# kensung-lab/hypo

Measured on AMD Instinct MI355X. Metric: polished windows/sec (whole node), higher is better.
Workload: dtype int16

## Files before the change

hypo_amd/csrc/poa_core.hpp:

```cpp
#pragma once
#include <math.h>
#include <type_traits>
#include "grp.hpp"
#include "../../include/hypo_gpu.h"

namespace hypo {
#ifdef HYPO_EMU_DBG
static unsigned long g_dbg_reason[16];
static unsigned long g_dbg_hist[64];
#define DBGH(d) do { if (g.lane == 0) g_dbg_hist[(d) < 63 ? (d) : 63]++; } while (0)
#else
#define DBGH(d) do { } while (0)
#endif

enum { MODE_NW = 1, MODE_LOV = 3, MODE_ROV = 4 };
enum { C_A = 0, C_C = 1, C_G = 2, C_T = 3, C_N = 4, C_J = 5, C_O = 6, C_NONE = 7 };
enum { PH_LOAD = 0, PH_DP = 1, PH_TRACE = 2, PH_ADD = 3, PH_TOPO = 4, PH_CONS = 5, PH_OUT = 6, PH_META = 7, PH_EXACT = 8, PH_N = 9 };
#if defined(HYPO_PHASE_TIMERS) && !defined(HYPO_EMU)
#define HYPO_TICK(k) do { const uint64_t t1_ = (uint64_t)clock64(); tphase[k] += t1_ - tlast; tlast = t1_; } while (0)
#define HYPO_TICK_RESET() do { tlast = (uint64_t)clock64(); } while (0)
#else
#define HYPO_TICK(k) do { } while (0)
#define HYPO_TICK_RESET() do { } while (0)
#endif

enum { RES_OK = 0, RES_OVERFLOW = 1, RES_UNDEFINED = 2, RES_CONS_OVERFLOW = 3, RES_UNSUPPORTED = 4, RES_INVALID = 5 };

struct PoaParams {
    const HypoWindow* windows;
    const uint8_t* draft4;
    const uint64_t* arm_off;
    const uint32_t* arm_len;
    const uint8_t* arms2;
    char* out_bases;
    const uint64_t* out_off;
    uint32_t* out_len;
    uint8_t* out_status;
    int sr_m, sr_n, sr_g, lr_m, lr_n, lr_g;
    uint64_t n_arms, draft4_bytes, arms2_bytes;
    int flags;
};
enum { POA_NATIVE_KLOV = 1, POA_MIN_CLASS_SHIFT = 8 };

#ifdef HYPO_EMU
struct PoaParamRef {
    const PoaParams* p;
    HD const PoaParams* operator->() const { return p; }
};
#else
struct PoaParamRef {
    typedef const PoaParams __attribute__((address_space(4)))* cptr;
    cptr p;
    HD cptr operator->() const { cptr q = p; asm volatile("" : "+s"(q)); return q; }
};
#endif

#ifndef HYPO_EXACT
#define HYPO_EXACT 1
#endif
#define HYPO_EXACT_WIDE 1
#ifndef HYPO_ONE_SUB
#define HYPO_ONE_SUB 1
#endif
#ifndef HYPO_ONE_SUB_ROV
#define HYPO_ONE_SUB_ROV 1
#endif
#ifndef HYPO_TOPO_INSERT
#define HYPO_TOPO_INSERT 1
#endif
#ifndef HYPO_DEFER_META
#define HYPO_DEFER_META 1
#endif
#define HYPO_PACKED 1
template <int GW_, int CPL_, int LCAP_, int NMAX_, int KIN_, int DIRCELLS_, int RINGCELLS_, int ARMBYTES_,
// ... 107 lines not shown
    static constexpr bool NIB = Cfg::NIB;
    static constexpr int NEG = -(1 << 29);
    static constexpr bool PK = Cfg::PACKED;
    static_assert(!PK || Cfg::NIB, "packed rows store nibble codes");
    static_assert(!PK || (int)sizeof(score_t) * Cfg::RINGCELLS >= Cfg::STK * (int)sizeof(id_t), "packed classes: the DFS stack fits the score ring");
    static constexpr int DIR_FAST = NIB ? 15 : 0xFF;
    static constexpr int DIR_HORIZ = NIB ? 14 : 0xFE;
    HD static int dir_diag(int p) { return NIB ? p : (p << 1); }
    HD static int dir_vert(int p) { return NIB ? 7 + p : ((p << 1) | 1); }
    HD static bool is_vert(int d) { return NIB ? d >= 7 : (d & 1); }
    HD static int dir_pred(int d) { return NIB ? (d >= 7 ? d - 7 : d) : (d >> 1); }

    static constexpr int pow2_of(int x) { return x & -x; }
    struct alignas(pow2_of((int)sizeof(score_t) * CPL)) Pack { score_t v[CPL]; };
    struct alignas(pow2_of(NIB ? CPL / 2 : CPL)) DPack { uint8_t v[NIB ? CPL / 2 : CPL]; };
    HD static uint32_t seq_ent(uint32_t src, uint32_t len, bool head, bool tail, int mode, bool , int where) {
        const uint32_t mc = mode == MODE_NW ? 0u : (mode == MODE_LOV ? 1u : 2u);
        return (src & 0x3fffu) | (len << 16) | ((head ? 1u : 0u) << 26) | ((tail ? 1u : 0u) << 27) | (mc << 28) |
               ((uint32_t)where << 30);
    }

    const Grp<GW>& g;
    const PoaParamRef P;
    score_t* ring; uint8_t* dir; uint32_t* rowmeta; uint32_t* seqtab; wt_t* inw; int16_t* posnode;
    id_t *inp, *al, *r2n, *n2r, *stack;
    uint8_t *code, *nin, *nout, *nal, *mark, *seq, *armbuf;
    uint8_t* sidx;
    id_t* pathnodes; uint32_t* pathoff; uint16_t *pathlen, *pathmult, *msa; uint32_t* dstcnt; uint8_t* consbuf; id_t* predrows; score_t* ring1;
    id_t *r2n_alt, *n2r_alt, *newid; int16_t* newslot;
    bool lazy_on; int n_new;
    int n_paths, path_used, head_first;
    int n_nodes; int L; bool topo_dirty; bool meta_dirty;
    int tb_steps; int tb_fv;
    bool last_changed;
    bool weights_done;
    bool threaded;
    enum { ST_CELLS = 0, ST_ALIGNS, ST_REUSED, ST_XHITS, ST_CSCORED, ST_CEXACT, ST_XT, ST_XH, ST_NEED, ST_CKIND, ST_CS, ST_CCHAIN0, ST_CPASS, ST_ARMB, ST_OLEN, ST_N,
           ST_LASTX = ST_CPASS,
           ST_MAXD = ST_N, ST_NSORT,
           ACC_CELLS, ACC_ALIGNS, ACC_ABYTES, ACC_REUSED, ACC_THR, ACC_CSCORED, ACC_CTHR, ACC_NOK, ACC_NESC, ACC_NFAIL, ACC_NCARRIED, ACC_END,
           NX_W0 = ACC_END, NX_OFF = NX_W0 + 10, NX_WIDX = NX_OFF + 4, NX_CARRY, CUR_STATIC, CUR_OFF, NX_END = CUR_OFF + 4 };
    static constexpr uint32_t NX_NONE = 0xffffffffu;
    static_assert(sizeof(HypoWindow) == 40, "the prefetch moves the descriptor as ten words");
    static_assert(NX_END <= Lay::STAT_BYTES / 4 && ST_N <= GW && GW >= 16, "stat block");
    enum { CARRY_NONE = 0, CARRY_BEFORE = 1, CARRY_UNSORTED = 2 };
    static constexpr int RES_OVERFLOW_CLEAN = 64;
    uint32_t* stat;
    HD void stat_add(int k, uint32_t v) const { if (g.lane == 0) stat[k] += v; }
    HD void stat_set(int k, uint32_t v) const { if (g.lane == 0) stat[k] = v; }
    HD uint32_t stat_get(int k) const { return stat[k]; }
#if defined(HYPO_PHASE_TIMERS) || defined(HYPO_EMU)
#define HYPO_DIAG(x) do { x; } while (0)
    uint32_t rows_done, topo_runs, cons_serial, rows_slow, exact_tries, guided_hits, rows_scored_n, topo_dfs, topo_fast;
    uint32_t one_sub_hits, cols_hits, topo_inserts, lazy_updates, tie_sorts;
#else
#define HYPO_DIAG(x) do { } while (0)
#endif
    uint64_t tphase[PH_N]; uint64_t tlast;

    HD Poa(const Grp<GW>& g_, const PoaParamRef& P_, char* mem, char* fast = nullptr, char* dirg = nullptr) : g(g_), P(P_) {
        ring = (score_t*)(mem + Lay::oRing); dir = Cfg::DIRG ? (uint8_t*)dirg : (uint8_t*)(mem + Lay::oDir);
        rowmeta = (uint32_t*)(mem + Lay::oRowmeta); seqtab = (uint32_t*)(mem + Lay::oSeqtab);
        inw = (wt_t*)(mem + Lay::oInw);
        constexpr bool HYB = Cfg::HYBRID;
        posnode = (int16_t*)(HYB ? fast + Lay::fPosnode : mem + Lay::oPosnode);
        inp = (id_t*)(mem + Lay::oInp); al = (id_t*)(mem + Lay::oAl);
        r2n = (id_t*)(mem + Lay::oR2n); n2r = (id_t*)(mem + Lay::oN2r);
        stack = (id_t*)(HYB ? fast + Lay::fPosnode : (PK ? mem + Lay::oRing : mem + Lay::oPosnode)); code = (uint8_t*)(mem + Lay::oCode);
        nin = (uint8_t*)(HYB ? fast + Lay::fNin : mem + Lay::oNin); nout = (uint8_t*)(mem + Lay::oNout);
        nal = (uint8_t*)(HYB ? fast + Lay::fNal : mem + Lay::oNal); mark = (uint8_t*)(HYB ? fast + Lay::fMark : mem + Lay::oMark);
        seq = (uint8_t*)(HYB ? fast + Lay::fSeq : mem + Lay::oSeq); armbuf = (uint8_t*)(mem + Lay::oArms);
        sidx = mark;
        pathnodes = (id_t*)(mem + Lay::oPathNodes); pathoff = (uint32_t*)(mem + Lay::oPathOff);
        pathlen = (uint16_t*)(mem + Lay::oPathLen); pathmult = (uint16_t*)(mem + Lay::oPathMult);
        msa = (uint16_t*)(mem + Lay::oMsa); dstcnt = (uint32_t*)(mem + Lay::oDst); consbuf = (uint8_t*)(mem + Lay::oCons);
        predrows = (id_t*)(mem + Lay::oPredRows);
        r2n_alt = (id_t*)(mem + Lay::oR2nAlt); n2r_alt = (id_t*)(mem + Lay::oN2rAlt); newid = (id_t*)(mem + Lay::oNewId); newslot = (int16_t*)(mem + Lay::oNewSlot);
        if constexpr (Cfg::LAZY_RING) {
            constexpr int oA = align_up<2>((NMAX + 1) * 2 > Cfg::STK * (int)sizeof(id_t) ? (NMAX + 1) * 2 : Cfg::STK * (int)sizeof(id_t));
            constexpr int oB = oA + NMAX * (int)sizeof(id_t), oC = oB + NMAX * (int)sizeof(id_t), oD = align_up<2>(oC + (Cfg::LMAX + 1) * (int)sizeof(id_t));
            static_assert(oD + (Cfg::LMAX + 1) * 2 <= (int)sizeof(score_t) * Cfg::RINGCELLS, "the lazy order's scratch fits the score ring");
            r2n_alt = (id_t*)(mem + Lay::oRing + oA); n2r_alt = (id_t*)(mem + Lay::oRing + oB); newid = (id_t*)(mem + Lay::oRing + oC); newslot = (int16_t*)(mem + Lay::oRing + oD);
        }
        lazy_on = false; n_new = 0; guide_len = -1; guide_mode = 0;
        stat = (uint32_t*)(HYB ? fast + Lay::fStat : mem + Lay::oStat);
        for (int t = g.lane; t < Lay::STAT_BYTES / 4; t += GW) stat[t] = 0;
        ring1 = (score_t*)(HYB ? fast + Lay::fRing1 : mem + Lay::oRing);
        n_paths = 0; path_used = 0; head_first = 0;
        n_nodes = 0; L = 0; topo_dirty = false; meta_dirty = true; tb_steps = 0; tb_fv = 0;
        last_changed = true; threaded = false;
        HYPO_DIAG(rows_done = 0; topo_runs = 0; cons_serial = 0; rows_slow = 0; exact_tries = 0; guided_hits = 0; rows_scored_n = 0; topo_dfs = 0; topo_fast = 0; one_sub_hits = 0; cols_hits = 0; topo_inserts = 0; lazy_updates = 0; tie_sorts = 0);
        for (int i = 0; i < PH_N; ++i) tphase[i] = 0;
        tlast = 0;
        HYPO_TICK_RESET();
    }

    Hook hk;
    HD void fetch_next() const {
        if constexpr (Hook::enabled) {
            g.sync();
            uint32_t a = 0;
            if (g.lane == 0) a = hk.claim();
            const uint32_t count = hk.count();
            const uint32_t idx = (uint32_t)g.shfl((int)a, 0);
            const uint32_t wn = idx < count ? hk.item(idx) : NX_NONE;
            a = wn;
            if (wn != NX_NONE) {
                if (g.lane < 10) a = ((const uint32_t*)(P->windows + wn))[g.lane];
                else if (g.lane < 14) a = ((const uint32_t*)(P->out_off + wn))[g.lane - 10];
                else if (g.lane == 15) a = idx >= hk.planned() ? hk.carry(wn) : 0u;
            }
            if (g.lane < 16) stat[NX_W0 + g.lane] = a;
            g.sync();
        }
    }
    HD void out_range(uint32_t w, uint64_t* o, uint64_t* cap) const {
        if constexpr (Hook::enabled) {
            const uint64_t o0 = (uint64_t)stat[CUR_OFF] | ((uint64_t)stat[CUR_OFF + 1] << 32), o1 = (uint64_t)stat[CUR_OFF + 2] | ((uint64_t)stat[CUR_OFF + 3] << 32);
            *o = o0; *cap = o1 - o0;
        } else { *o = P->out_off[w]; *cap = P->out_off[w + 1] - *o; }
    }

    HD int build_seqtab(const HypoWindow& W, bool is_long, int* n_seq_out, bool* added_out) {
        const uint32_t a0 = W.first_arm;
        const int ni = (int)W.n_internal, np = (int)W.n_prefix, ns = (int)W.n_suffix;
        const int narm = ni + np + ns;
        const int base = (ni == 0 || is_long) ? 1 : 0;
        if (narm + base > Cfg::SEQMAX) return RES_OVERFLOW;
        if ((int)W.draft_len + (is_long ? 0 : 2) > Cfg::LMAX && base) return RES_OVERFLOW;
        g.sync();
        if (base && g.lane == 0) seqtab[0] = seq_ent(0, W.draft_len, !is_long, !is_long, MODE_NW, true, 2);
        bool over = false, any_len = false, bad = false;
        uint32_t armb = 0;
        if constexpr (STAGE_FUSED) {
            if (!is_long) return build_seqtab_fused(W, base, narm, n_seq_out, added_out);
        }
        for (int t = g.lane; t < narm; t += GW) {
            int a, mode; bool head, tail;
            if (is_long) { a = t; mode = MODE_NW; head = false; tail = false; }
            else if (t < ni) { a = t; mode = MODE_NW; head = true; tail = true; }
            else if (t < ni + np) { a = ni + (np - 1 - (t - ni)); mode = MODE_LOV; head = true; tail = false; }
            else { a = t; mode = MODE_ROV; head = false; tail = true; }
            const uint32_t len = P->arm_len[a0 + a];
            { const uint64_t ao = P->arm_off[a0 + a], ab = P->arms2_bytes; if (ao > ab || ((uint64_t)len + 3) / 4 > ab - ao) { bad = true; continue; } }
// ... 2415 lines not shown
                int c = 0;
                for (int q = 0; q < pl; ++q) {
                    const int v = pn[q];
                    const int mv = msa[v];
                    while (c < len && (int)msa[path[len - 1 - c]] < mv) ++c;
                    if (c >= len) break;
                    const int cn = path[len - 1 - c];
                    if ((int)msa[cn] == mv && code[v] == code[cn]) atomic_inc(&dstcnt[c], mult);
                }
            }
            g.sync();
            int o = 0;
            for (int base = 0; base < len; base += GW) {
                const int c = base + g.lane;
                const bool keep = c < len && counter_load(&dstcnt[c]) >= thr;
                const uint64_t kb = g.ballot(keep);
                const int cd = c < len ? (int)code[path[len - 1 - c]] : 0;
                g.sync();
                if (keep) consbuf[o + popc64(kb & ((1ull << g.lane) - 1ull))] = (uint8_t)cd;
                o += popc64(kb);
            }
            conslen = o;
            g.sync();
            HYPO_TICK(PH_CONS);
        }
        uint64_t oo, cap; out_range(w, &oo, &cap);
        if ((uint64_t)conslen > cap) { finish(w, HYPO_ST_CONS_OVERFLOW, (uint32_t)conslen); return RES_OK; }
        for (int t = g.lane; t < conslen; t += GW) P->out_bases[oo + t] = "ACGTNJO"[consbuf[t]];
        finish(w, HYPO_ST_OK, (uint32_t)conslen);
        return RES_OK;
    }

    HD void finish(uint32_t w, int status, uint32_t len) const {
        if (g.lane == 0) { P->out_len[w] = len; P->out_status[w] = (uint8_t)status; if constexpr (Hook::enabled) stat[ST_OLEN] = len; }
    }
    HD int emit_draft(uint32_t w, const uint8_t* d4, int dlen) const {
        uint64_t o, cap; out_range(w, &o, &cap);
        if ((uint64_t)dlen > cap) { finish(w, HYPO_ST_CONS_OVERFLOW, (uint32_t)dlen); return RES_OK; }
        for (int t = g.lane; t < dlen; t += GW) {
            int c = (d4[t >> 1] >> (4 - 4 * (t & 1))) & 15;
            P->out_bases[o + t] = "ACGTN"[c < 4 ? c : 4];
        }
        finish(w, HYPO_ST_OK, (uint32_t)dlen);
        return RES_OK;
    }

    HD int run_short(uint32_t w, const HypoWindow& W, const uint8_t* carry_in) {
        const int m = P->sr_m, n = P->sr_n, gp = P->sr_g;
        const uint8_t* d4 = P->draft4 + W.draft_off;
        n_nodes = 0; topo_dirty = false; meta_dirty = true;
        lazy_on = Cfg::LAZY && !Cfg::LAZY_RING && !(P->flags & POA_NATIVE_KLOV);
        stat_set(ST_NSORT, 0u);
        int n_seq = 0; bool added = false;
        int rc = build_seqtab(W, false, &n_seq, &added);
        if (rc != RES_OK) return rc;
        bool prev_aligned = false;
        int s = 0;
        int chain0_in = 0;
        if (carry_in) {
            if ((rc = restore(carry_in, &s, &chain0_in)) != RES_OK) return rc;
            if (s > n_seq) return RES_INVALID;
            if (topo_dirty) { if ((rc = toposort()) != RES_OK) return rc; HYPO_DIAG(topo_runs += 1); HYPO_TICK(PH_TOPO); }
            if constexpr (Cfg::LAZY_RING) { if (!(P->flags & POA_NATIVE_KLOV)) lazy_on = true; }
        }
        int chain0 = chain0_in;
        auto project = [&](int rc_) -> int {
            if (rc_ == RES_OVERFLOW && s > 0 && n_nodes > 0) {
                const int grown = n_nodes - chain0 > 0 ? n_nodes - chain0 : 0;
                if (g.lane == 0) {
                    stat[ST_NEED] = (uint32_t)(n_nodes + (int)(((int64_t)grown * (n_seq - s) + s - 1) / s) + 4);
                    const uint32_t kind = stat[ST_CKIND];
                    stat[ST_CS] = (uint32_t)(kind == CARRY_UNSORTED ? s : s - 1);
                    stat[ST_CCHAIN0] = (uint32_t)(chain0 ? chain0 : (kind == CARRY_UNSORTED ? n_nodes : 0));
                }
            } else stat_set(ST_CKIND, CARRY_NONE);
            g.sync();
            return rc_;
        };
        while (s < n_seq) {
            if (prev_aligned && !last_changed && tb_steps != 0 && tb_fv == 0) {
                int c = 0;
                while (s < n_seq && same_as_previous(s)) { ++c; ++s; }
                if (c) {
                    if (g.lane == 0) { stat[ST_CELLS] += (uint32_t)(c * (n_nodes + 1) * (L + 1)); stat[ST_ALIGNS] += c; stat[ST_REUSED] += c; }
                    if ((rc = readd_alignment(c)) != RES_OK) return project(rc);
                    HYPO_TICK(PH_ADD);
                    if (s >= n_seq) break;
                }
            }
            int mode;
            if ((rc = load_seq(W, s, &mode)) != RES_OK) return rc;
            ++s;
            if (L == 0) { prev_aligned = false; continue; }
            if ((rc = add_sequence_step(mode, m, n, gp)) != RES_OK) return project(rc);
            if (chain0 == 0) chain0 = n_nodes;
            prev_aligned = true;
        }
        if (!added) return emit_draft(w, d4, (int)W.draft_len);
        if constexpr (Cfg::LAZY) {
            if (lazy_on && n_nodes > 0) { if ((rc = toposort()) != RES_OK) return rc; meta_dirty = true; HYPO_TICK(PH_TOPO); }
            lazy_on = false;
        }
        int16_t* path;
        const int len = consensus(&path);
        HYPO_TICK(PH_CONS);
        if (len < 2) return RES_UNDEFINED;
        const int olen = len - 2;
        uint64_t o, cap; out_range(w, &o, &cap);
        if ((uint64_t)olen > cap) { finish(w, HYPO_ST_CONS_OVERFLOW, (uint32_t)olen); return RES_OK; }
        for (int t = g.lane; t < olen; t += GW) P->out_bases[o + t] = "ACGTNJO"[code[path[len - 2 - t]]];
        finish(w, HYPO_ST_OK, (uint32_t)olen);
        HYPO_TICK(PH_OUT);
        return RES_OK;
    }

    HD int run(uint32_t w, const uint8_t* carry_in = nullptr) {
        const HypoWindow W = P->windows[w];
        return run_window(w, W, carry_in);
    }
    HD int run_window(uint32_t w, const HypoWindow& W, const uint8_t* carry_in) {
        last_changed = true;
        g.sync();
        if (g.lane < ST_N) stat[g.lane] = 0;
        g.sync();
        HYPO_DIAG(rows_done = 0; topo_runs = 0; cons_serial = 0; rows_slow = 0; exact_tries = 0; guided_hits = 0; rows_scored_n = 0; topo_dfs = 0; topo_fast = 0; one_sub_hits = 0; cols_hits = 0; topo_inserts = 0; lazy_updates = 0; tie_sorts = 0);
        n_paths = 0; path_used = 0; head_first = 0; L = 0; tb_steps = 0; tb_fv = 0;
        lazy_on = false; n_new = 0; guide_len = -1;
        for (int i = 0; i < PH_N; ++i) tphase[i] = 0;
        HYPO_TICK_RESET();
        const uint32_t ne = W.n_internal + W.n_prefix + W.n_suffix;
        if ((uint64_t)W.n_internal + W.n_prefix + W.n_suffix > P->n_arms || (uint64_t)W.first_arm + ne > P->n_arms ||
            W.draft_off > P->draft4_bytes || ((uint64_t)W.draft_len + 1) / 2 > P->draft4_bytes - W.draft_off) return RES_INVALID;
        if constexpr (Hook::enabled) {
            if ((W.n_empty > ne || ne < 2) && g.lane == 0) {
                uint32_t a = 0;
                HYPO_NOUNROLL
                for (uint32_t t = 0; t < ne; ++t) a += (P->arm_len[W.first_arm + t] + 3) >> 2;
                stat[ST_ARMB] = a;
            }
        }
        if (W.n_empty > ne) { finish(w, HYPO_ST_OK, 0); return RES_OK; }
        if (ne < 2) return emit_draft(w, P->draft4 + W.draft_off, (int)W.draft_len);
        if (W.type != HYPO_WIN_SHORT) {
            if (Cfg::PATHCAP == 0) return RES_UNSUPPORTED;
            return run_long(w, W);
        }
        const int rc = run_short(w, W, carry_in);
        if (g.lane == 0) stat[ST_CPASS] = (rc == RES_OVERFLOW && carry_in && stat[ST_CKIND] == CARRY_NONE) ? 1u : 0u;
        g.sync();
        return rc;
    }
};

}
```

hypo_amd/csrc/poa_kernel.hip:

```cpp
#include <hip/hip_runtime.h>
#include <hip/hip_ext.h>
#include <atomic>
#include <stdio.h>
#include <stdlib.h>
#include "poa_classes.hpp"
#include "poa_kernel.hpp"
#include "poa_giant.hpp"
#include <cstring>

namespace hypo {

struct ClassLimits { int lmax, nmax, dircells, ringcells, seqmax, cpl; };

template <class Cfg> __host__ __device__ constexpr ClassLimits limits_of() {
    return ClassLimits{Cfg::LMAX, Cfg::NMAX, Cfg::DIRCELLS, Cfg::RINGCELLS, Cfg::SEQMAX, Cfg::CPL};
}

constexpr int PLAN_THREADS = 256;
constexpr int PLAN_STAGE = 4096;
constexpr int PLAN_AHEAD = 4;
constexpr int PLAN_LANES = 4;
constexpr int PLAN_WPB = PLAN_THREADS / PLAN_LANES;

__device__ __forceinline__ uint32_t plan_key_from(const HypoWindow& W, uint32_t maxarm, uint32_t changes, bool* trivial, int min_short_class = 0) {
    const uint32_t narm = W.n_internal + W.n_prefix + W.n_suffix;
    uint32_t maxlen = (W.n_internal == 0 || W.type != HYPO_WIN_SHORT) ? W.draft_len + 2 : 0;
    if (narm) maxlen = maxarm + 2 > maxlen ? maxarm + 2 : maxlen;
#define HYPO_PLAN_GROW_Q 2
    const uint32_t slack = maxlen / 16 + 3, grow = changes * HYPO_PLAN_GROW_Q / 4 + 3;
    const uint32_t est_nodes = maxlen + (grow > slack ? grow : slack);
    const ClassLimits lim[kNumPoaClasses] = {
#define HYPO_LIM(ID, CFG) limits_of<CFG>(),
        HYPO_FOR_EACH_CLASS(HYPO_LIM)
#undef HYPO_LIM
    };
    int cls = kNumPoaClasses - 1;
    for (int c = 0; c < kNumPoaClasses; ++c) {
        const uint32_t S = (maxlen + 1 + lim[c].cpl - 1) / lim[c].cpl * lim[c].cpl;
        if ((int)maxlen <= lim[c].lmax && (int)est_nodes <= lim[c].nmax && (int)narm + 1 <= lim[c].seqmax &&
            (uint64_t)est_nodes * S <= (uint64_t)lim[c].dircells && lim[c].ringcells / (int)S >= 6) { cls = c; break; }
    }
    if (W.type != HYPO_WIN_SHORT && cls < kFirstLongClass) cls = kFirstLongClass;
    if (W.type == HYPO_WIN_SHORT && cls < min_short_class) cls = min_short_class;
    *trivial = W.n_empty > narm || narm < 2;
    const uint32_t cost = *trivial ? 0u : maxlen * (narm + 1);
    const uint32_t cmax = (uint32_t)lim[cls].lmax * (uint32_t)(lim[cls].seqmax < 64 ? lim[cls].seqmax : 64);
    uint32_t b = (uint32_t)(((uint64_t)cost * kPlanBuckets) / (cmax ? cmax : 1));
    b = b >= (uint32_t)kPlanBuckets ? kPlanBuckets - 1 : b;
    return (uint32_t)cls * kPlanBuckets + (kPlanBuckets - 1 - b);
}

__global__ void __launch_bounds__(PLAN_THREADS)
poa_plan_count_kernel(PoaParams P, PoaQueues Q, uint32_t n_windows, uint32_t* ticket ) {
    __shared__ uint32_t lens[PLAN_STAGE];
    __shared__ uint32_t hist[kNumPoaClasses * kPlanBuckets];
    __shared__ uint32_t amin, amax, ntriv, drawn;
    const uint32_t w = blockIdx.x * PLAN_WPB + threadIdx.x / PLAN_LANES, sub = threadIdx.x % PLAN_LANES;
    for (int i = threadIdx.x; i < kNumPoaClasses * kPlanBuckets; i += PLAN_THREADS) hist[i] = 0;
    if (threadIdx.x == 0) { amin = 0xffffffffu; amax = 0; ntriv = 0; }
    __syncthreads();
    HypoWindow W{};
    uint32_t narm = 0;
    if (w < n_windows) {
        W = P.windows[w];
        narm = W.n_internal + W.n_prefix + W.n_suffix;
        if ((uint64_t)W.n_internal + W.n_prefix + W.n_suffix + (uint64_t)W.first_arm > P.n_arms) { narm = 0; W.n_internal = W.n_prefix = W.n_suffix = 0; }
        if (narm && sub == 0) { atomicMin(&amin, W.first_arm); atomicMax(&amax, W.first_arm + narm); }
    }
    __syncthreads();
    const uint32_t a0 = amin, a1 = amax;
    const bool staged = a1 > a0 && a1 - a0 <= (uint32_t)PLAN_STAGE;
    if (staged) for (uint32_t i = threadIdx.x; i < a1 - a0; i += PLAN_THREADS) lens[i] = P.arm_len[a0 + i];
    __syncthreads();
    {
        uint32_t maxarm = 0;
        if (staged) { for (uint32_t a = sub; a < narm; a += PLAN_LANES) { const uint32_t l = lens[W.first_arm - a0 + a]; maxarm = l > maxarm ? l : maxarm; } }
        else { for (uint32_t a = sub; a < narm; a += PLAN_LANES) { const uint32_t l = P.arm_len[W.first_arm + a]; maxarm = l > maxarm ? l : maxarm; } }
        uint32_t changes = 0;
        if (W.type == HYPO_WIN_SHORT && (uint64_t)W.first_arm + narm <= P.n_arms) {
            auto arm_at = [&](uint32_t a, uint32_t* l_out) -> const uint8_t* {
                const uint32_t l = staged ? lens[W.first_arm - a0 + a] : P.arm_len[W.first_arm + a];
                const uint64_t o = P.arm_off[W.first_arm + a];
                const uint32_t nb = (l + 3) / 4;
                *l_out = l;
                return (o <= P.arms2_bytes && nb <= P.arms2_bytes - o) ? P.arms2 + o : nullptr;
            };
            for (uint32_t a0l = 1 + sub; a0l < W.n_internal; a0l += PLAN_AHEAD * PLAN_LANES) {
                const uint8_t *p[PLAN_AHEAD], *q[PLAN_AHEAD];
                uint32_t l[PLAN_AHEAD], pl[PLAN_AHEAD];
#pragma unroll
                for (int u = 0; u < PLAN_AHEAD; ++u) {
                    const uint32_t a = a0l + (uint32_t)u * PLAN_LANES;
                    p[u] = q[u] = nullptr; l[u] = pl[u] = 0;
                    if (a < W.n_internal) { p[u] = arm_at(a, &l[u]); q[u] = arm_at(a - 1, &pl[u]); }
                }
#pragma unroll
                for (int u = 0; u < PLAN_AHEAD; ++u) {
                    const uint32_t nb = (l[u] + 3) / 4;
                    if (p[u] && q[u] && l[u] == pl[u]) {
                        typedef uint64_t __attribute__((aligned(1))) u64u;
                        uint32_t b = 0;
                        for (; b + 8 <= nb; b += 8) {
                            uint64_t x = *(const u64u*)(p[u] + b) ^ *(const u64u*)(q[u] + b);
                            x |= x >> 4; x |= x >> 2; x |= x >> 1;
                            changes += (uint32_t)__popcll(x & 0x0101010101010101ull);
                        }
                        for (; b < nb; ++b) changes += p[u][b] != q[u][b];
                    }
                }
            }
        }
        for (int d = 1; d < PLAN_LANES; d <<= 1) {
            changes += (uint32_t)__shfl_xor((int)changes, d, PLAN_LANES);
            const uint32_t om = (uint32_t)__shfl_xor((int)maxarm, d, PLAN_LANES);
            maxarm = om > maxarm ? om : maxarm;
        }
        if (w < n_windows && sub == 0) {
            bool trivial;
            const uint32_t key = plan_key_from(W, maxarm, changes, &trivial, (P.flags >> POA_MIN_CLASS_SHIFT) & 3);
            Q.keys[w] = (uint16_t)key;
            Q.carry[w] = 0;
            P.out_status[w] = 0xff;
            P.out_len[w] = 0;
            Q.items[(size_t)3 * Q.stride + w] = kQueueUnpublished;
            atomicAdd(&hist[key], 1u);
            if (trivial) atomicAdd(&ntriv, 1u);
        }
    }
    __syncthreads();
    for (int i = threadIdx.x; i < kNumPoaClasses * kPlanBuckets; i += PLAN_THREADS)
        if (hist[i]) { const uint32_t before = atomicAdd(&Q.hist[i], hist[i]); HYPO_ARRIVED(before); }
    if (threadIdx.x == 0 && ntriv) atomicAdd((unsigned long long*)&Q.stats->n_trivial, (unsigned long long)ntriv);
// ... 59 lines not shown
    __device__ __forceinline__ uint32_t carry(uint32_t w) const { return HYPO_LD_DEV(&ka()->Q.carry[w]); }
};
#define HYPO_PREFETCH_NEXT 1

#define HYPO_C4_WAVES 2
template <class Cfg> struct PoaMinWaves { static constexpr int value = Cfg::HYBRID ? HYPO_C4_WAVES : (Cfg::DIRG ? 4 : (Cfg::GW < 64 ? 3 : 1)); };
constexpr uint64_t kPollLimitTicks = 50u * 1000u * 1000u;
template <class Cfg, bool USE_LDS, bool POLL = false>
__global__ void __launch_bounds__(64, PoaMinWaves<Cfg>::value) poa_class_kernel(PoaKArgs ) {
    extern __shared__ __attribute__((aligned(16))) char smem[];
    const PoaKArgPtr ka = (PoaKArgPtr)__builtin_amdgcn_kernarg_segment_ptr();
    constexpr int GW = Cfg::GW;
    constexpr int GPW = 64 / GW;
    const int wl = (int)(threadIdx.x & 63);
    const int grp = wl / GW;
    Grp<GW> g{wl & (GW - 1)};
    char* mem = USE_LDS ? smem + (size_t)grp * PoaLayout<Cfg>::BYTES
                        : fresh(ka)->scratch + ((size_t)blockIdx.x * GPW + grp) * PoaLayout<Cfg>::BYTES;
    char* fast = smem + (size_t)grp * PoaLayout<Cfg>::FAST_BYTES;
    char* dirg = Cfg::DIRG ? fresh(ka)->dirg + ((size_t)blockIdx.x * GPW + grp) * PoaLayout<Cfg>::DIRG_BYTES : nullptr;
    const int cls = fresh(ka)->cls;
    if (!POLL && USE_LDS && wl == 0) atomicAdd((unsigned long long*)(fresh(ka)->Q.work + cls), 0ull - (unsigned long long)wall_clock64());
    if (!POLL && USE_LDS && cls == 0 && blockIdx.x == 0 && wl == 0) fresh(ka)->Q.work[6] = (uint64_t)GW;
    const uint32_t count = POLL ? 0u : *fresh(ka)->bound;
    const uint32_t planned = fresh(ka)->Q.planned[cls];
    const PoaParamRef P{&ka->P};
    constexpr bool PF = HYPO_PREFETCH_NEXT && USE_LDS && !POLL;
    typedef typename std::conditional<PF, Poa<Cfg, PoaPrefetch>, Poa<Cfg>>::type PoaT;
    uint64_t cells = 0, aligns = 0, abytes = 0, n_reused = 0, n_thr = 0, c_scored = 0, c_thr = 0;
    uint32_t n_ok = 0, n_esc = 0, n_fail = 0, n_carried = 0;
    uint32_t carry_in = 0;
#ifdef HYPO_PHASE_TIMERS
    uint64_t tph[PH_N] = {0, 0, 0, 0, 0, 0, 0, 0, 0};
    uint64_t dbg[20] = {0, 0, 0, 0, 0, 0, 0, 0, 0, 0, 0, 0, 0, 0, 0, 0, 0, 0, 0, 0};
    const uint64_t tstart = (uint64_t)clock64();
#endif
    auto account = [&](PoaT& poa, uint32_t w, int rc) {
        uint32_t* const stt = poa.stat;
        if constexpr (USE_LDS) {
            if (g.lane == 0) {
                if (rc == RES_OK) {
                    stt[PoaT::ACC_CELLS] += stt[PoaT::ST_CELLS]; stt[PoaT::ACC_ALIGNS] += stt[PoaT::ST_ALIGNS];
                    stt[PoaT::ACC_REUSED] += stt[PoaT::ST_REUSED]; stt[PoaT::ACC_THR] += stt[PoaT::ST_XHITS];
                }
                stt[PoaT::ACC_CSCORED] += stt[PoaT::ST_CSCORED]; stt[PoaT::ACC_CTHR] += stt[PoaT::ST_CEXACT];
            }
        } else {
            if (rc == RES_OK) { cells += stt[PoaT::ST_CELLS]; aligns += stt[PoaT::ST_ALIGNS]; n_reused += stt[PoaT::ST_REUSED]; n_thr += stt[PoaT::ST_XHITS]; }
            c_scored += stt[PoaT::ST_CSCORED]; c_thr += stt[PoaT::ST_CEXACT];
        }
#ifdef HYPO_PHASE_TIMERS
        for (int i = 0; i < PH_N; ++i) tph[i] += poa.tphase[i];
        dbg[0] += poa.rows_done; dbg[1] += stt[PoaT::ST_ALIGNS] - stt[PoaT::ST_REUSED]; dbg[2] += stt[PoaT::ST_REUSED]; dbg[3] += poa.topo_runs; dbg[4] += poa.cons_serial; dbg[5] += poa.rows_slow; dbg[6] += poa.exact_tries; dbg[7] += stt[PoaT::ST_XHITS]; dbg[8] += poa.guided_hits; dbg[9] += poa.rows_scored_n; dbg[10] += poa.topo_dfs; dbg[11] += poa.topo_fast; dbg[12] += poa.one_sub_hits; dbg[13] += poa.cols_hits; dbg[14] += poa.topo_inserts; dbg[15] += poa.lazy_updates; dbg[16] += poa.tie_sorts;
#endif
        if (rc == RES_OK) {
            if (g.lane == 0) {
                if constexpr (PF) {
                    stt[PoaT::ACC_ABYTES] += stt[PoaT::CUR_STATIC] + stt[PoaT::ST_OLEN] + stt[PoaT::ST_ARMB];
                    stt[PoaT::ACC_NOK] += 1;
                } else {
                    const HypoWindow W = P->windows[w];
                    const uint32_t narm = W.n_internal + W.n_prefix + W.n_suffix;
                    uint32_t a = (uint32_t)((W.draft_len + 1) / 2 + 16 + 8 * (1 + narm) + P->out_len[w]);
                    const uint32_t* alen = P->arm_len;
                    for (uint32_t t = 0; t < narm; ++t) a += (alen[W.first_arm + t] + 3) / 4;
                    if constexpr (USE_LDS) { stt[PoaT::ACC_ABYTES] += a; stt[PoaT::ACC_NOK] += 1; } else abytes += a;
                }
            }
            if constexpr (!USE_LDS) ++n_ok;
        } else if ((rc == RES_OVERFLOW || rc == RES_UNSUPPORTED) && cls + 1 < kNumPoaClasses) {
            const int to = cls < kRequeueClass ? kRequeueClass : cls + 1;
            uint32_t cv = 0;
            if (rc == RES_OVERFLOW && stt[PoaT::ST_CKIND] != PoaT::CARRY_NONE) {
                const uint32_t sz16 = poa.spill_size() >> 4;
                const uint32_t cap16 = fresh(ka)->Q.spill_cap16;
                uint32_t off = 0xffffffffu;
#ifdef HYPO_PHASE_TIMERS
                const uint64_t tc0 = (uint64_t)clock64();
#endif
                if (g.lane == 0) {
                    const unsigned long long got = atomicAdd(fresh(ka)->Q.spill_used, (unsigned long long)sz16);
                    if (got + sz16 <= (unsigned long long)cap16) off = (uint32_t)got;
                }
                off = (uint32_t)g.shfl((int)off, 0);
#ifdef HYPO_PHASE_TIMERS
                const uint64_t tc1 = (uint64_t)clock64();
                dbg[18] += tc1 - tc0;
#endif
                if (off != 0xffffffffu) {
                    poa.spill((uint8_t*)fresh(ka)->Q.spill + (size_t)off * 16);
#ifdef HYPO_PHASE_TIMERS
                    dbg[19] += (uint64_t)clock64() - tc1;
#endif
                    cv = off + 1;
                    if constexpr (USE_LDS) { if (g.lane == 0) stt[PoaT::ACC_NCARRIED] += 1; } else ++n_carried;
                }
            } else if (rc == RES_OVERFLOW && stt[PoaT::ST_CPASS]) cv = carry_in;
            if (g.lane == 0) {
                HYPO_ST_DEV(&fresh(ka)->Q.carry[w], cv);
                HYPO_RELEASE_STORES();
                const uint32_t slot = atomicAdd(&fresh(ka)->Q.count[to], 1u);
                __hip_atomic_store(&fresh(ka)->Q.items[(size_t)to * fresh(ka)->Q.stride + slot], w, __ATOMIC_RELAXED, __HIP_MEMORY_SCOPE_AGENT);
            }
            if constexpr (USE_LDS) { if (g.lane == 0) stt[PoaT::ACC_NESC] += 1; } else ++n_esc;
        } else if (rc == RES_OVERFLOW || rc == RES_UNSUPPORTED) {
            if (g.lane == 0) {
                const uint32_t slot = atomicAdd(&fresh(ka)->Q.count[kGiantClass], 1u);
                __hip_atomic_store(&fresh(ka)->Q.items[slot], w, __ATOMIC_RELAXED, __HIP_MEMORY_SCOPE_AGENT);
            }
        } else {
            if (g.lane == 0) {
                P->out_len[w] = 0;
                P->out_status[w] = (uint8_t)(rc == RES_UNDEFINED ? HYPO_ST_UNDEFINED : (rc == RES_INVALID ? HYPO_ST_INVALID : HYPO_ST_CAPACITY));
            }
            if constexpr (USE_LDS) { if (g.lane == 0) stt[PoaT::ACC_NFAIL] += 1; } else ++n_fail;
        }
    };
    auto aload = [](const uint32_t* p) -> uint32_t { return __hip_atomic_load(p, __ATOMIC_RELAXED, __HIP_MEMORY_SCOPE_AGENT); };
    auto dequeue = [&](uint32_t* w) -> bool {
        uint32_t idx = 0;
        if constexpr (POLL) {
            const uint32_t* const cnt = fresh(ka)->Q.count + cls;
            const uint32_t* const done = fresh(ka)->Q.done;
            const uint32_t expected = fresh(ka)->expected;
            auto producers_done = [&]() -> bool {
                uint32_t d = 0;
                for (int c = 0; c < cls; ++c) d += aload(done + c);
                return d >= expected;
            };
            uint64_t t0 = wall_clock64();
            for (;;) {
                const bool final_queue = producers_done();
                if (final_queue) __builtin_amdgcn_fence(__ATOMIC_ACQUIRE, "agent");
                const uint32_t h = aload(fresh(ka)->head);
                const uint32_t c = aload(cnt);
                if (final_queue && h >= c) return false;
                if (h < c) {
                    uint32_t got = kQueueUnpublished;
                    if (g.lane == 0 && atomicCAS(fresh(ka)->head, h, h + 1u) == h) got = h;
                    got = (uint32_t)g.shfl((int)got, 0);
                    if (got == kQueueUnpublished) continue;
                    idx = got;
                    const uint32_t* const slot = fresh(ka)->Q.items + (size_t)cls * fresh(ka)->Q.stride + idx;
                    for (;;) {
                        const uint32_t v = aload(slot);
                        if (v != kQueueUnpublished) { *w = v; break; }
                        __builtin_amdgcn_s_sleep(8);
                    }
                    __builtin_amdgcn_fence(__ATOMIC_ACQUIRE, "workgroup");
                    break;
                }
                if (wall_clock64() - t0 > kPollLimitTicks) return false;
                __builtin_amdgcn_s_sleep(127);
            }
        } else {
            if (__atomic_load_n(fresh(ka)->head, __ATOMIC_RELAXED) >= count) return false;
            if (g.lane == 0) idx = atomicAdd(fresh(ka)->head, 1u);
            idx = (uint32_t)g.shfl((int)idx, 0);
            if (idx >= count) return false;
            *w = fresh(ka)->Q.items[(size_t)cls * fresh(ka)->Q.stride + idx];
        }
        carry_in = idx >= planned ? HYPO_LD_DEV(&fresh(ka)->Q.carry[*w]) : 0u;
        return true;
    };
    PoaT poa(g, P, mem, fast, dirg);
    if constexpr (PF) {
        uint32_t* const stt = poa.stat;
        poa.fetch_next();
        for (;;) {
            const uint32_t w = (uint32_t)g.uniform((int)stt[PoaT::NX_WIDX]);
            if (w == PoaT::NX_NONE) break;
            HypoWindow W;
            { uint32_t* const wd = (uint32_t*)&W; HYPO_UNROLL for (int i = 0; i < 10; ++i) wd[i] = (uint32_t)g.uniform((int)stt[PoaT::NX_W0 + i]); }
            carry_in = (uint32_t)g.uniform((int)stt[PoaT::NX_CARRY]);
            const uint32_t oc = g.lane < 4 ? stt[PoaT::NX_OFF + g.lane] : 0u;
            g.sync();
            if (g.lane < 4) stt[PoaT::CUR_OFF + g.lane] = oc;
            if (g.lane == 4) stt[PoaT::CUR_STATIC] = (uint32_t)((W.draft_len + 1) / 2 + 16 + 8 * (1 + W.n_internal + W.n_prefix + W.n_suffix));
            const int rc = poa.run_window(w, W, carry_in ? (const uint8_t*)fresh(ka)->Q.spill + (size_t)(carry_in - 1) * 16 : nullptr);
#ifdef HYPO_PHASE_TIMERS
            const uint64_t ta = (uint64_t)clock64();
#endif
            account(poa, w, rc);
#ifdef HYPO_PHASE_TIMERS
            const uint64_t tb = (uint64_t)clock64();
#endif
            poa.fetch_next();
#ifdef HYPO_PHASE_TIMERS
            dbg[17] += tb - ta;
#endif
        }
    } else {
        uint32_t w;
        while (dequeue(&w)) account(poa, w, poa.run(w, carry_in ? (const uint8_t*)fresh(ka)->Q.spill + (size_t)(carry_in - 1) * 16 : nullptr));
    }
    if (g.lane == 0) {
        HypoPoaStats* st = fresh(ka)->Q.stats;
        if constexpr (USE_LDS) {
            const uint32_t* const stt = poa.stat;
            cells = stt[PoaT::ACC_CELLS]; aligns = stt[PoaT::ACC_ALIGNS]; abytes = stt[PoaT::ACC_ABYTES]; n_reused = stt[PoaT::ACC_REUSED];
            n_thr = stt[PoaT::ACC_THR]; c_scored = stt[PoaT::ACC_CSCORED]; c_thr = stt[PoaT::ACC_CTHR]; n_ok = stt[PoaT::ACC_NOK];
            n_esc = stt[PoaT::ACC_NESC]; n_fail = stt[PoaT::ACC_NFAIL]; n_carried = stt[PoaT::ACC_NCARRIED];
        }
        atomicAdd((unsigned long long*)&st->n_carried, (unsigned long long)n_carried);
        atomicAdd((unsigned long long*)&st->n_class[cls], (unsigned long long)n_ok);
        atomicAdd((unsigned long long*)&st->n_escalated, (unsigned long long)n_esc);
        atomicAdd((unsigned long long*)&st->n_failed, (unsigned long long)n_fail);
        atomicAdd((unsigned long long*)&st->dp_cells, (unsigned long long)cells);
        atomicAdd((unsigned long long*)&st->n_alignments, (unsigned long long)aligns);
        atomicAdd((unsigned long long*)&st->alg_bytes[cls], (unsigned long long)abytes);
        atomicAdd((unsigned long long*)&st->n_reused, (unsigned long long)n_reused);
        atomicAdd((unsigned long long*)&st->n_threaded, (unsigned long long)n_thr);
        atomicAdd((unsigned long long*)&st->cells_scored, (unsigned long long)c_scored);
        atomicAdd((unsigned long long*)&st->cells_threaded, (unsigned long long)c_thr);
#ifdef HYPO_PHASE_TIMERS
        static_assert(kNumPoaClasses * 32 * 8 <= 2048 - 512 && PH_N + 2 + 20 <= 32, "phase block of the header");
        unsigned long long* ph = (unsigned long long*)((char*)fresh(ka)->Q.count + kPoaHdrPhase) + (size_t)cls * 32;
        for (int i = 0; i < PH_N; ++i) atomicAdd(&ph[i], (unsigned long long)tph[i]);
        atomicAdd(&ph[PH_N], (unsigned long long)((uint64_t)clock64() - tstart));
        atomicAdd(&ph[PH_N + 1], 1ull);
        for (int i = 0; i < 20; ++i) atomicAdd(&ph[PH_N + 2 + i], (unsigned long long)dbg[i]);
#endif
        HYPO_RELEASE_STORES();
        atomicAdd(fresh(ka)->Q.done + cls, 1u);
    }
    if (!POLL && USE_LDS && wl == 0) atomicAdd((unsigned long long*)(fresh(ka)->Q.work + cls), (unsigned long long)wall_clock64());
}

struct GiantKArgs { PoaParams P; PoaQueues Q; char* arena; uint64_t slice_bytes; };
__global__ void __launch_bounds__(64) poa_giant_kernel(GiantKArgs ) {
    typedef const GiantKArgs __attribute__((address_space(4)))* KPtr;
    const KPtr ka = (KPtr)__builtin_amdgcn_kernarg_segment_ptr();
    if (blockIdx.x == 0 && threadIdx.x < 8) {
        PoaPinned* const host = ka->Q.host;
        __hip_atomic_store(host->final_count + threadIdx.x, ka->Q.count[threadIdx.x], __ATOMIC_RELAXED, __HIP_MEMORY_SCOPE_SYSTEM);
        __hip_atomic_store((unsigned long long*)host->work + threadIdx.x, (unsigned long long)ka->Q.work[threadIdx.x], __ATOMIC_RELAXED, __HIP_MEMORY_SCOPE_SYSTEM);
    }
    const uint32_t pending = ka->Q.count[kGiantClass];
    if (pending == 0) return;
    const Grp<64> g{(int)(threadIdx.x & 63)};
    const PoaParamRef P{&ka->P};
    uint64_t cells = 0, aligns = 0, abytes = 0;
// ... 375 lines not shown
```

Measured before the change: 70.80 million.

## Stage packed arm bytes in LDS for plan-count change counting, widen plan blocks

The plan-count kernel now stages arm lengths and offsets as 16-bit values, plus a byte window of packed arm sequences, in a shared pool. Short-window adjacent-arm difference counting then runs from LDS using alignbyte word reads instead of global loads. The block size and stage size are doubled. It also adds optional cycle timers around build_seqtab and a profiling script. This gives more LDS per block and adds validity checks with a fallback path when offsets or lengths do not fit.

New measurement: 72.10 million (median of 6 runs). 1.8% higher.

```diff
diff --git a/hypo_amd/csrc/poa_core.hpp b/hypo_amd/csrc/poa_core.hpp
--- a/hypo_amd/csrc/poa_core.hpp
+++ b/hypo_amd/csrc/poa_core.hpp
@@ -19,7 +19,9 @@
 #if defined(HYPO_PHASE_TIMERS) && !defined(HYPO_EMU)
 #define HYPO_TICK(k) do { const uint64_t t1_ = (uint64_t)clock64(); tphase[k] += t1_ - tlast; tlast = t1_; } while (0)
 #define HYPO_TICK_RESET() do { tlast = (uint64_t)clock64(); } while (0)
+#define HYPO_CYCLES(x) do { x; } while (0)
 #else
+#define HYPO_CYCLES(x) do { } while (0)
 #define HYPO_TICK(k) do { } while (0)
 #define HYPO_TICK_RESET() do { } while (0)
 #endif
@@ -233,6 +235,7 @@
 #if defined(HYPO_PHASE_TIMERS) || defined(HYPO_EMU)
 #define HYPO_DIAG(x) do { x; } while (0)
     uint32_t rows_done, topo_runs, cons_serial, rows_slow, exact_tries, guided_hits, rows_scored_n, topo_dfs, topo_fast;
+    uint64_t seqtab_cycles;
     uint32_t one_sub_hits, cols_hits, topo_inserts, lazy_updates, tie_sorts;
 #else
 #define HYPO_DIAG(x) do { } while (0)
@@ -270,7 +273,7 @@
         n_paths = 0; path_used = 0; head_first = 0;
         n_nodes = 0; L = 0; topo_dirty = false; meta_dirty = true; tb_steps = 0; tb_fv = 0;
         last_changed = true; threaded = false;
-        HYPO_DIAG(rows_done = 0; topo_runs = 0; cons_serial = 0; rows_slow = 0; exact_tries = 0; guided_hits = 0; rows_scored_n = 0; topo_dfs = 0; topo_fast = 0; one_sub_hits = 0; cols_hits = 0; topo_inserts = 0; lazy_updates = 0; tie_sorts = 0);
+        HYPO_DIAG(rows_done = 0; topo_runs = 0; cons_serial = 0; rows_slow = 0; exact_tries = 0; guided_hits = 0; rows_scored_n = 0; topo_dfs = 0; topo_fast = 0; one_sub_hits = 0; cols_hits = 0; topo_inserts = 0; lazy_updates = 0; tie_sorts = 0; seqtab_cycles = 0);
         for (int i = 0; i < PH_N; ++i) tphase[i] = 0;
         tlast = 0;
         HYPO_TICK_RESET();
@@ -2792,7 +2795,9 @@
         lazy_on = Cfg::LAZY && !Cfg::LAZY_RING && !(P->flags & POA_NATIVE_KLOV);
         stat_set(ST_NSORT, 0u);
         int n_seq = 0; bool added = false;
+        HYPO_CYCLES(seqtab_cycles -= (uint64_t)clock64());
         int rc = build_seqtab(W, false, &n_seq, &added);
+        HYPO_CYCLES(seqtab_cycles += (uint64_t)clock64());
         if (rc != RES_OK) return rc;
         bool prev_aligned = false;
         int s = 0;
@@ -2863,7 +2868,7 @@
         g.sync();
         if (g.lane < ST_N) stat[g.lane] = 0;
         g.sync();
-        HYPO_DIAG(rows_done = 0; topo_runs = 0; cons_serial = 0; rows_slow = 0; exact_tries = 0; guided_hits = 0; rows_scored_n = 0; topo_dfs = 0; topo_fast = 0; one_sub_hits = 0; cols_hits = 0; topo_inserts = 0; lazy_updates = 0; tie_sorts = 0);
+        HYPO_DIAG(rows_done = 0; topo_runs = 0; cons_serial = 0; rows_slow = 0; exact_tries = 0; guided_hits = 0; rows_scored_n = 0; topo_dfs = 0; topo_fast = 0; one_sub_hits = 0; cols_hits = 0; topo_inserts = 0; lazy_updates = 0; tie_sorts = 0; seqtab_cycles = 0);
         n_paths = 0; path_used = 0; head_first = 0; L = 0; tb_steps = 0; tb_fv = 0;
         lazy_on = false; n_new = 0; guide_len = -1;
         for (int i = 0; i < PH_N; ++i) tphase[i] = 0;
diff --git a/hypo_amd/csrc/poa_kernel.hip b/hypo_amd/csrc/poa_kernel.hip
--- a/hypo_amd/csrc/poa_kernel.hip
+++ b/hypo_amd/csrc/poa_kernel.hip
@@ -16,8 +16,9 @@
     return ClassLimits{Cfg::LMAX, Cfg::NMAX, Cfg::DIRCELLS, Cfg::RINGCELLS, Cfg::SEQMAX, Cfg::CPL};
 }
 
-constexpr int PLAN_THREADS = 256;
-constexpr int PLAN_STAGE = 4096;
+constexpr int PLAN_THREADS = 512;
+constexpr int PLAN_STAGE = 8192;
+constexpr int PLAN_POOL = 36864;
 constexpr int PLAN_AHEAD = 4;
 constexpr int PLAN_LANES = 4;
 constexpr int PLAN_WPB = PLAN_THREADS / PLAN_LANES;
@@ -52,12 +53,14 @@
 
 __global__ void __launch_bounds__(PLAN_THREADS)
 poa_plan_count_kernel(PoaParams P, PoaQueues Q, uint32_t n_windows, uint32_t* ticket ) {
-    __shared__ uint32_t lens[PLAN_STAGE];
+    __shared__ __attribute__((aligned(16))) uint8_t pool[PLAN_POOL];
     __shared__ uint32_t hist[kNumPoaClasses * kPlanBuckets];
-    __shared__ uint32_t amin, amax, ntriv, drawn;
+    __shared__ uint32_t amin, amax, ntriv, drawn, unfit, bend;
+    static_assert(PLAN_POOL % 32 == 0 && PLAN_POOL >= 4 * PLAN_STAGE + 4096 && 4 * PLAN_STAGE + 65536 > PLAN_POOL, "lengths, offsets and a useful byte window");
+    static_assert(4 * (PLAN_POOL + 4 * kNumPoaClasses * kPlanBuckets + 1024) <= 160 * 1024 && 4 * PLAN_THREADS <= 2048, "four workgroups per CU, with room");
     const uint32_t w = blockIdx.x * PLAN_WPB + threadIdx.x / PLAN_LANES, sub = threadIdx.x % PLAN_LANES;
     for (int i = threadIdx.x; i < kNumPoaClasses * kPlanBuckets; i += PLAN_THREADS) hist[i] = 0;
-    if (threadIdx.x == 0) { amin = 0xffffffffu; amax = 0; ntriv = 0; }
+    if (threadIdx.x == 0) { amin = 0xffffffffu; amax = 0; ntriv = 0; unfit = 0; bend = 0; }
     __syncthreads();
     HypoWindow W{};
     uint32_t narm = 0;
@@ -69,15 +72,65 @@
     }
     __syncthreads();
     const uint32_t a0 = amin, a1 = amax;
-    const bool staged = a1 > a0 && a1 - a0 <= (uint32_t)PLAN_STAGE;
-    if (staged) for (uint32_t i = threadIdx.x; i < a1 - a0; i += PLAN_THREADS) lens[i] = P.arm_len[a0 + i];
+    const bool in_stage = a1 > a0 && a1 - a0 <= (uint32_t)PLAN_STAGE;
+    const uint32_t npad = in_stage ? (a1 - a0 + 7) & ~7u : 0;
+    uint16_t* const lens = (uint16_t*)pool;
+    uint16_t* const offs = lens + npad;
+    uint8_t* const bytes = pool + 4 * npad;
+    const uint32_t bleft = PLAN_POOL - 4 * npad - 16, bcap = bleft < 65520u ? bleft : 65520u;
+    uint64_t base = 0;
+    if (in_stage) {
+        base = P.arm_off[a0] & ~(uint64_t)15;
+        uint32_t bad = ((uintptr_t)P.arms2 & 15) ? 2u : 0u, end = 0;
+        for (uint32_t i = threadIdx.x; i < a1 - a0; i += PLAN_THREADS) {
+            const uint32_t l = P.arm_len[a0 + i];
+            const uint64_t o = P.arm_off[a0 + i];
+            const uint32_t nb = (l + 3) / 4;
+            if (l > 0xffffu) bad |= 1u;
+            if (!(o <= P.arms2_bytes && nb <= P.arms2_bytes - o) || o < base || o - base + nb > bcap) bad |= 2u;
+            else end = (uint32_t)(o - base) + nb > end ? (uint32_t)(o - base) + nb : end;
+            lens[i] = (uint16_t)l;
+            offs[i] = (uint16_t)(o - base);
+        }
+        if (bad) atomicOr(&unfit, bad);
+        if (end) atomicMax(&bend, end);
+    }
+    __syncthreads();
+    const bool staged = in_stage && !(unfit & 1u);
+    const bool packed = in_stage && !unfit;
+    if (packed) {
+        const uint32_t nchunk = (bend + 15) / 16;
+        for (uint32_t c = threadIdx.x; c <= nchunk; c += PLAN_THREADS) {
+            const uint64_t g = base + (uint64_t)16 * c;
+            uint32_t v[4] = {0, 0, 0, 0};
+            if (c == nchunk) { }
+            else if (g + 16 <= P.arms2_bytes) { const uint4 q = *(const uint4*)(P.arms2 + g); v[0] = q.x; v[1] = q.y; v[2] = q.z; v[3] = q.w; }
+            else for (uint32_t k = 0; k < 16 && g + k < P.arms2_bytes; ++k) v[k / 4] |= (uint32_t)P.arms2[g + k] << (8 * (k % 4));
+            *(uint4*)(bytes + 16 * c) = make_uint4(v[0], v[1], v[2], v[3]);
+        }
+    }
     __syncthreads();
     {
         uint32_t maxarm = 0;
         if (staged) { for (uint32_t a = sub; a < narm; a += PLAN_LANES) { const uint32_t l = lens[W.first_arm - a0 + a]; maxarm = l > maxarm ? l : maxarm; } }
         else { for (uint32_t a = sub; a < narm; a += PLAN_LANES) { const uint32_t l = P.arm_len[W.first_arm + a]; maxarm = l > maxarm ? l : maxarm; } }
         uint32_t changes = 0;
-        if (W.type == HYPO_WIN_SHORT && (uint64_t)W.first_arm + narm <= P.n_arms) {
+        if (packed && W.type == HYPO_WIN_SHORT) {
+            const uint32_t* const words = (const uint32_t*)bytes;
+            auto word_at = [&](uint32_t o) { return __builtin_amdgcn_alignbyte(words[o / 4 + 1], words[o / 4], o & 3); };
+            const uint32_t f = W.first_arm - a0;
+            for (uint32_t a = 1 + sub; a < W.n_internal; a += PLAN_LANES) {
+                const uint32_t l = lens[f + a];
+                if (l != lens[f + a - 1]) continue;
+                const uint32_t nb = (l + 3) / 4, po = offs[f + a], qo = offs[f + a - 1];
+                for (uint32_t b = 0; b < nb; b += 4) {
+                    uint32_t x = word_at(po + b) ^ word_at(qo + b);
+                    if (nb - b < 4) x &= (1u << (8 * (nb - b))) - 1;
+                    x |= x >> 4; x |= x >> 2; x |= x >> 1;
+                    changes += (uint32_t)__popc(x & 0x01010101u);
+                }
+            }
+        } else if (W.type == HYPO_WIN_SHORT && (uint64_t)W.first_arm + narm <= P.n_arms) {
             auto arm_at = [&](uint32_t a, uint32_t* l_out) -> const uint8_t* {
                 const uint32_t l = staged ? lens[W.first_arm - a0 + a] : P.arm_len[W.first_arm + a];
                 const uint64_t o = P.arm_off[W.first_arm + a];
@@ -243,6 +296,9 @@
 #ifdef HYPO_PHASE_TIMERS
         for (int i = 0; i < PH_N; ++i) tph[i] += poa.tphase[i];
         dbg[0] += poa.rows_done; dbg[1] += stt[PoaT::ST_ALIGNS] - stt[PoaT::ST_REUSED]; dbg[2] += stt[PoaT::ST_REUSED]; dbg[3] += poa.topo_runs; dbg[4] += poa.cons_serial; dbg[5] += poa.rows_slow; dbg[6] += poa.exact_tries; dbg[7] += stt[PoaT::ST_XHITS]; dbg[8] += poa.guided_hits; dbg[9] += poa.rows_scored_n; dbg[10] += poa.topo_dfs; dbg[11] += poa.topo_fast; dbg[12] += poa.one_sub_hits; dbg[13] += poa.cols_hits; dbg[14] += poa.topo_inserts; dbg[15] += poa.lazy_updates; dbg[16] += poa.tie_sorts;
+#ifdef HYPO_OPEN_TIMERS
+        dbg[19] += poa.seqtab_cycles;
+#endif
 #endif
         if (rc == RES_OK) {
             if (g.lane == 0) {
@@ -276,12 +332,16 @@
                 off = (uint32_t)g.shfl((int)off, 0);
 #ifdef HYPO_PHASE_TIMERS
                 const uint64_t tc1 = (uint64_t)clock64();
+#ifndef HYPO_OPEN_TIMERS
                 dbg[18] += tc1 - tc0;
+#endif
 #endif
                 if (off != 0xffffffffu) {
                     poa.spill((uint8_t*)fresh(ka)->Q.spill + (size_t)off * 16);
 #ifdef HYPO_PHASE_TIMERS
+#ifndef HYPO_OPEN_TIMERS
                     dbg[19] += (uint64_t)clock64() - tc1;
+#endif
 #endif
                     cv = off + 1;
                     if constexpr (USE_LDS) { if (g.lane == 0) stt[PoaT::ACC_NCARRIED] += 1; } else ++n_carried;
@@ -379,6 +439,9 @@
             poa.fetch_next();
 #ifdef HYPO_PHASE_TIMERS
             dbg[17] += tb - ta;
+#ifdef HYPO_OPEN_TIMERS
+            dbg[18] += (uint64_t)clock64() - tb;
+#endif
 #endif
         }
     } else {
diff --git a/profiles/open_phases.py b/profiles/open_phases.py
--- /dev/null
+++ b/profiles/open_phases.py
@@ -0,0 +1,37 @@
+#!/usr/bin/env python3
+import os
+import sys
+
+import numpy as np
+
+ROOT = os.path.dirname(os.path.dirname(os.path.abspath(__file__)))
+sys.path.insert(0, ROOT)
+import torch
+from hypo_amd import capi, sim
+
+NP = 9
+
+
+def main():
+    gpu = capi.HypoGpu(0, path=sys.argv[1])
+    n = int(sys.argv[2]) if len(sys.argv) > 2 else 97078
+    sub = float(sys.argv[3]) if len(sys.argv) > 3 else 0.002
+    db = gpu.device_batch(sim.window_batch(n, seed=1000, read_sub=sub))
+    for _ in range(2):
+        db.run()
+    torch.cuda.synchronize()
+    st = db.stats()
+    ph = db.workspace[512:512 + 6 * 32 * 8].cpu().numpy().view(np.uint64).reshape(6, 32)
+    print(f"# {n} windows, read_sub={sub}, concurrent schedule, last of two calls; cycles of the wave's clock64(), summed over waves, per window of the class")
+    print("class  windows  lifetime/window  fetch_next  build_seqtab  both  share of lifetime  load_seq  account")
+    for c in range(3):
+        nw = st["n_class"][c]
+        if not nw or not ph[c, NP + 1]:
+            continue
+        D = NP + 2
+        life, fetch, seqtab, load, acct = (float(ph[c, i]) / nw for i in (NP, D + 18, D + 19, 0, D + 17))
+        print(f"{c:5d}  {nw:7d}  {life:15.0f}  {fetch:10.0f}  {seqtab:12.0f}  {fetch + seqtab:4.0f}  {100 * (fetch + seqtab) / life:16.2f}%  {load:8.0f}  {acct:7.0f}")
+
+
+if __name__ == "__main__":
+    main()
```
